# hyperledger-labs/bdls

Measured on AMD Instinct MI355X. Metric: P-256 ECDSA verifies/sec (fused SHA-256, bit-exact vs Go crypto/ecdsa + Fabric low-S), higher is better.
Workload: dtype u32; 1 GPU; BASELINE config 2: 1048576 records/GPU, 256B messages, 65536 distinct keys, 1/16 corrupted, fused SHA-256; records_per_gpu=1048576, records_total=1048576, msg_len=256, nkeys=65536, corrupt_den=16, parallelism=shard1 (no collective)

## Files before the change

### bdls_amd/csrc/bdls_hip.cpp

```cpp
#include <hip/hip_runtime.h>

#include <algorithm>
#include <cctype>
#include <atomic>
#include <chrono>
#include <condition_variable>
#include <deque>
#include <memory>
#include <cstdio>
#include <cstdlib>
#include <cstring>
#include <functional>
#include <mutex>
#include <string>
#include <unordered_map>
#include <thread>
#include <vector>

#include "../../include/bdls_hip.h"
#include "verify.h"
#include "verify384.h"
#include "pack.h"
#include "shard.h"

// ... 448 lines not shown

std::vector<Dev*> all_devs() {
  std::lock_guard<std::mutex> g(g_mu);
  return g_devs;
}

uint32_t env_block(const char* name, uint32_t dflt) {
  const char* e = getenv(name);
  const long v = e ? atol(e) : 0L;
  return (v == 64 || v == 128 || v == 256) ? (uint32_t)v : dflt;
}

int env_route() {
  const char* e = getenv("BH_ROUTE");
  if (!e) return 0;
  if (!strcmp(e, "ladder")) return 2;
  if (!strcmp(e, "noreg")) return 1;
  return 0;
}

bh::LaunchOpts launch_opts(size_t m, uint32_t flags) {
  bh::LaunchOpts o;
  static const long env_chunk = [] {
    const char* e = getenv("BH_INV_CHUNK");
    return e ? atol(e) : 0L;
  }();
  o.inv_chunk = env_chunk > 0 ? (uint32_t)std::min<long>(env_chunk, 64)
                              : (uint32_t)std::max<size_t>(1, std::min<size_t>(16, m / 131072));
  o.keep = (flags & BH_F_KEEP_KEYS) != 0;
  o.min_uses = o.keep ? 2u : bh::kMinUses;
  o.min_batch = o.keep ? 0u : bh::kKeyTableMinBatch;
  o.wide = bh::wide_for(m);
  o.wide_block = env_block("BH_WIDE_BLOCK", 256);
  return o;
}

bh::BatchIn slice(const bh_batch* b, size_t base, uint32_t flags) {
  return bh::BatchIn{b->pub + base * 64, b->sig, b->sig_off + base, b->sig_len + base,
                     b->msg, b->msg_off + base, b->msg_len + base, flags};
}
bh::BdlsIn slice(const bh_bdls_batch* b, size_t base, uint32_t flags) {
  return bh::BdlsIn{b->xy + base * 64, b->r, b->r_off + base, b->r_len + base,
                    b->s, b->s_off + base, b->s_len + base,
// ... 50 lines not shown
  }
  for (size_t base = 0; base < n; base += chunk) {
    const size_t m = std::min(chunk, n - base);
    bh::Work w;
    bh::Plan pl;
    int rc = carve_work(d, m, &w, &pl, false, lane > 0 ? L.ws : nullptr);
    if (rc) return rc;
    bh::LaunchOpts o = launch_opts(m, flags);
    {
      const char* e = getenv("BH_LL");
      o.ll_tables = !(e && atoi(e) == 0);
    }
    const int route = env_route();
    bh::KeyReg g = d.reg[curve].g;
    if (route >= 1 && !(flags & BH_F_KEEP_KEYS)) g.cap = 0;
    if (route >= 2 && !(flags & BH_F_KEEP_KEYS)) o.min_uses = UINT32_MAX;
    o.aux = L.aux;
    o.ev_fork = L.fork;
    o.ev_join = L.join;
    o.records_ready = records_ready;
    if (lane >= 0 && d.build_staggered && lanes() > 1) {
      const uint32_t nl = lanes();
      o.ev_build_wait = lane_ref(d, (int)((lane + nl - 1) % nl)).build;
      o.ev_build_done = L.build;
    }
    hipEvent_t* ev = t ? d.ev : nullptr;
    if (!t && d.defer) {
      if (d.ev_used == d.ev_pool.size()) {
        d.ev_pool.emplace_back(7, nullptr);
        for (auto& e : d.ev_pool.back()) HIPCHK(hipEventCreate(&e));
      }
// ... 1942 lines not shown
```

### bdls_amd/csrc/curve_consts.h

```cpp
#pragma once
#include <stdint.h>
namespace bh {
struct Fp_p256 {
  static constexpr uint32_t m[8] = {0xffffffffu, 0xffffffffu, 0xffffffffu, 0x00000000u, 0x00000000u, 0x00000000u, 0x00000001u, 0xffffffffu};
  static constexpr uint32_t n0 = 0x00000001u;
  static constexpr uint32_t r1[8] = {0x00000001u, 0x00000000u, 0x00000000u, 0xffffffffu, 0xffffffffu, 0xffffffffu, 0xfffffffeu, 0x00000000u};
  static constexpr uint32_t r2[8] = {0x00000003u, 0x00000000u, 0xffffffffu, 0xfffffffbu, 0xfffffffeu, 0xffffffffu, 0xfffffffdu, 0x00000004u};
  static constexpr uint32_t mm2[8] = {0xfffffffdu, 0xffffffffu, 0xffffffffu, 0x00000000u, 0x00000000u, 0x00000000u, 0x00000001u, 0xffffffffu};
  static constexpr uint32_t r3[8] = {0x0000000au, 0xfffffffdu, 0xfffffff7u, 0xffffffedu, 0xfffffffcu, 0x00000005u, 0x00000001u, 0x00000018u};
  static constexpr int32_t s30[9] = {1073741823, 1073741823, 1073741823, 63, 0, 0, 4096, 1073725440, 65535};
  static constexpr uint32_t inv30 = 0x3fffffffu;
};
struct Fn_p256 {
  static constexpr uint32_t m[8] = {0xfc632551u, 0xf3b9cac2u, 0xa7179e84u, 0xbce6faadu, 0xffffffffu, 0xffffffffu, 0x00000000u, 0xffffffffu};
  static constexpr uint32_t n0 = 0xee00bc4fu;
  static constexpr uint32_t r1[8] = {0x039cdaafu, 0x0c46353du, 0x58e8617bu, 0x43190552u, 0x00000000u, 0x00000000u, 0xffffffffu, 0x00000000u};
  static constexpr uint32_t r2[8] = {0xbe79eea2u, 0x83244c95u, 0x49bd6fa6u, 0x4699799cu, 0x2b6bec59u, 0x2845b239u, 0xf3d95620u, 0x66e12d94u};
  static constexpr uint32_t mm2[8] = {0xfc63254fu, 0xf3b9cac2u, 0xa7179e84u, 0xbce6faadu, 0xffffffffu, 0xffffffffu, 0x00000000u, 0xffffffffu};
  static constexpr uint32_t r3[8] = {0x0b65a624u, 0xac8ebec9u, 0x0c0555c9u, 0x111f28aeu, 0x6ba5e93fu, 0x2543b924u, 0x6407be65u, 0x503a54e7u};
  static constexpr int32_t s30[9] = {1013130577, 250030859, 830072911, 968797033, 1073741756, 1073741823, 4095, 1073725440, 65535};
  static constexpr uint32_t inv30 = 0x11ff43b1u;
};
struct Cv_p256 {
  static constexpr uint32_t b_m[8] = {0x29c4bddfu, 0xd89cdf62u, 0x78843090u, 0xacf005cdu, 0xf7212ed6u, 0xe5a220abu, 0x04874834u, 0xdc30061du};
// ... 9 lines not shown
  static constexpr uint32_t p[9] = {0x3fffffffu, 0x3fffffffu, 0x3fffffffu, 0x0000003fu, 0x00000000u, 0x00000000u, 0x00001000u, 0x3fffc000u, 0x0000ffffu};
  static constexpr uint32_t n0 = 0x00000001u;
  static constexpr uint32_t r1[9] = {0x00004000u, 0x00000000u, 0x00000000u, 0x3ff00000u, 0x3fffffffu, 0x3fffffffu, 0x3bffffffu, 0x0fffffffu, 0x00000000u};
  static constexpr uint32_t r2[9] = {0x30000000u, 0x00000000u, 0x00000000u, 0x3ffffffcu, 0x3fffffbfu, 0x3fffffbfu, 0x3fffffffu, 0x3ffff7ffu, 0x00004fffu};
  static constexpr uint32_t r3[9] = {0x00006000u, 0x0000a000u, 0x3fff4000u, 0x3fdfffffu, 0x3fb7ffffu, 0x3fcfffffu, 0x3b7fffffu, 0x18ffffffu, 0x00000000u};
  using M32 = Fp_p256;
  static constexpr uint32_t k32[9] = {0x7fffffe0u, 0x7ffffffeu, 0x7ffffffeu, 0x400007feu, 0x3fffffffu, 0x3fffffffu, 0x4001ffffu, 0x7ff7ffffu, 0x001ffffeu};
  static constexpr uint32_t k64[9] = {0x7fffffc0u, 0x7ffffffeu, 0x7ffffffeu, 0x40000ffeu, 0x3fffffffu, 0x3fffffffu, 0x4003ffffu, 0x7fefffffu, 0x003ffffeu};
  static constexpr uint32_t b_m[9] = {0x2f77f70cu, 0x1f6229c4u, 0x02436273u, 0x1cc9c543u, 0x35ab3c01u, 0x2bf7212eu, 0x1025c882u, 0x1e0b7483u, 0x00000187u};
  static constexpr uint32_t gx_m[9] = {0x050f0624u, 0x30d418a9u, 0x1805e79cu, 0x1fc475dbu, 0x041d6ea5u, 0x2b776225u, 0x1985adccu, 0x2bdc755cu, 0x000017ddu};
  static constexpr uint32_t gy_m[9] = {0x1582a15cu, 0x1357ce95u, 0x117377c9u, 0x0e434a9eu, 0x0962d2aeu, 0x08dd21f3u, 0x1535e21au, 0x0aaf85d8u, 0x00007fc6u};
  static constexpr uint32_t pm2[8] = {0xfffffffdu, 0xffffffffu, 0xffffffffu, 0x00000000u, 0x00000000u, 0x00000000u, 0x00000001u, 0xffffffffu};
  static constexpr int a_is_minus3 = 1;
  static constexpr int sparse_p256 = 1;
};
struct Fp_k1 {
  static constexpr uint32_t m[8] = {0xfffffc2fu, 0xfffffffeu, 0xffffffffu, 0xffffffffu, 0xffffffffu, 0xffffffffu, 0xffffffffu, 0xffffffffu};
  static constexpr uint32_t n0 = 0xd2253531u;
  static constexpr uint32_t r1[8] = {0x000003d1u, 0x00000001u, 0x00000000u, 0x00000000u, 0x00000000u, 0x00000000u, 0x00000000u, 0x00000000u};
  static constexpr uint32_t r2[8] = {0x000e90a1u, 0x000007a2u, 0x00000001u, 0x00000000u, 0x00000000u, 0x00000000u, 0x00000000u, 0x00000000u};
  static constexpr uint32_t mm2[8] = {0xfffffc2du, 0xfffffffeu, 0xffffffffu, 0xffffffffu, 0xffffffffu, 0xffffffffu, 0xffffffffu, 0xffffffffu};
  static constexpr uint32_t r3[8] = {0x3795f671u, 0x002bb1e3u, 0x00000b73u, 0x00000001u, 0x00000000u, 0x00000000u, 0x00000000u, 0x00000000u};
  static constexpr int32_t s30[9] = {1073740847, 1073741819, 1073741823, 1073741823, 1073741823, 1073741823, 1073741823, 1073741823, 65535};
  static constexpr uint32_t inv30 = 0x2ddacacfu;
};
struct Fn_k1 {
  static constexpr uint32_t m[8] = {0xd0364141u, 0xbfd25e8cu, 0xaf48a03bu, 0xbaaedce6u, 0xfffffffeu, 0xffffffffu, 0xffffffffu, 0xffffffffu};
  static constexpr uint32_t n0 = 0x5588b13fu;
  static constexpr uint32_t r1[8] = {0x2fc9bebfu, 0x402da173u, 0x50b75fc4u, 0x45512319u, 0x00000001u, 0x00000000u, 0x00000000u, 0x00000000u};
  static constexpr uint32_t r2[8] = {0x67d7d140u, 0x896cf214u, 0x0e7cf878u, 0x741496c2u, 0x5bcd07c6u, 0xe697f5e4u, 0x81c69bc5u, 0x9d671cd5u};
// ... 16 lines not shown
  static constexpr uint32_t p[9] = {0x3ffffc2fu, 0x3ffffffbu, 0x3fffffffu, 0x3fffffffu, 0x3fffffffu, 0x3fffffffu, 0x3fffffffu, 0x3fffffffu, 0x0000ffffu};
  static constexpr uint32_t n0 = 0x12253531u;
  static constexpr uint32_t r1[9] = {0x00f44000u, 0x00010000u, 0x00000000u, 0x00000000u, 0x00000000u, 0x00000000u, 0x00000000u, 0x00000000u, 0x00000000u};
  static constexpr uint32_t r2[9] = {0x10000000u, 0x0003a428u, 0x000007a2u, 0x00000004u, 0x00000000u, 0x00000000u, 0x00000000u, 0x00000000u, 0x00000000u};
  static constexpr uint32_t r3[9] = {0x00000000u, 0x1f671000u, 0x2c78cde5u, 0x0b73002bu, 0x00040000u, 0x00000000u, 0x00000000u, 0x00000000u, 0x00000000u};
  using M32 = Fp_k1;
  static constexpr uint32_t k32[9] = {0x7fff85e0u, 0x7fffff7eu, 0x7ffffffeu, 0x7ffffffeu, 0x7ffffffeu, 0x7ffffffeu, 0x7ffffffeu, 0x7ffffffeu, 0x001ffffeu};
  static constexpr uint32_t k64[9] = {0x7fff0bc0u, 0x7ffffefeu, 0x7ffffffeu, 0x7ffffffeu, 0x7ffffffeu, 0x7ffffffeu, 0x7ffffffeu, 0x7ffffffeu, 0x003ffffeu};
  static constexpr uint32_t b_m[9] = {0x06adc000u, 0x00070000u, 0x00000000u, 0x00000000u, 0x00000000u, 0x00000000u, 0x00000000u, 0x00000000u, 0x00000000u};
  static constexpr uint32_t gx_m[9] = {0x08b83460u, 0x2e5ae1feu, 0x1b6f5cd8u, 0x15329bc6u, 0x2708c78au, 0x0033fd12u, 0x225e7d23u, 0x3e9089f4u, 0x00007990u};
  static constexpr uint32_t gy_m[9] = {0x2bbe38ffu, 0x26d3a317u, 0x1936c57au, 0x15d1f1dcu, 0x0da37f17u, 0x1aac19c1u, 0x19c2dad6u, 0x3d4a582du, 0x0000e147u};
  static constexpr uint32_t pm2[8] = {0xfffffc2du, 0xfffffffeu, 0xffffffffu, 0xffffffffu, 0xffffffffu, 0xffffffffu, 0xffffffffu, 0xffffffffu};
  static constexpr int a_is_minus3 = 0;
  static constexpr int sparse_p256 = 0;
};
}
```

### bdls_amd/csrc/ec30.h

```cpp
#pragma once
#include "fp30.h"

namespace bh {

struct J30 {
  uint32_t X[9], Y[9], Z[9];
};

BH_HD void j_copy(J30& r, const J30& p) {
  f_copy(r.X, p.X);
  f_copy(r.Y, p.Y);
  f_copy(r.Z, p.Z);
}

BH_HD void j_sel(J30& r, bool c, const J30& a, const J30& b) {
  f_sel(r.X, c, a.X, b.X);
  f_sel(r.Y, c, a.Y, b.Y);
  f_sel(r.Z, c, a.Z, b.Z);
}

template <class F>
BH_HD void j_dbl(J30& r, const J30& p) {
  if constexpr (F::a_is_minus3) {
    uint32_t delta[9], gamma[9], bt[9], t0[9], t1[9], u[9], alpha[9];
// ... 101 lines not shown
  f_mul<F>(w1, p.X, c);
  f_mul<F>(w2, q.X, c);
  f_sub<F, 64>(t2, p.Y, q.Y);
  f_sqr<F>(d, t2);
  f_sub<F, 32>(t3, w1, w2);
  f_mul<F>(p.Y, p.Y, t3);
  f_sub2<F, 32>(r.X, d, w1, w2);
  f_sub<F, 64>(t3, w1, r.X);
  f_mul<F>(t3, t2, t3);
  f_sub<F, 32>(r.Y, t3, p.Y);
  f_mul<F>(r.Z, p.Z, t1);
  f_copy(p.X, w1);
  f_copy(p.Z, r.Z);
}

template <class F>
BH_HD bool j_degenerate(const uint32_t z3[9], const uint32_t rr[9], bool* same_y) {
  const bool degenerate = f_is_zero2<F>(z3);
  if (degenerate) {
    uint32_t t[9];
    f_reduce<F>(t, rr);
    uint32_t z = 0;
    for (int i = 0; i < 9; i++) z |= t[i];
    *same_y = (z == 0);
  } else {
    *same_y = false;
  }
  return degenerate;
}

template <class F, bool CO>
BH_HD bool j_add_impl(J30& r, J30* pz, const J30& p, const J30& q, bool neg, bool* same_y) {
  uint32_t z1z1[9], z2z2[9], u1[9], u2[9], s1[9], s2[9], h[9], rr[9], t[9], hh[9], hhh[9], w[9];
// ... 24 lines not shown
    f_copy(pz->Y, s1);
    f_copy(pz->Z, r.Z);
  }
  return j_degenerate<F>(r.Z, rr, same_y);
}

template <class F>
BH_HD bool j_add(J30& r, const J30& p, const J30& q, bool* same_y) {
  return j_add_impl<F, false>(r, nullptr, p, q, false, same_y);
}
template <class F>
BH_HD bool j_add_co(J30& r, J30& pz, const J30& p, const J30& q, bool* same_y, bool neg = false) {
  return j_add_impl<F, true>(r, &pz, p, q, neg, same_y);
}

template <class F, bool CO>
BH_HD bool j_madd_impl(J30& r, J30* pz, const J30& p, const uint32_t x2[9], const uint32_t y2[9],
                       bool neg, bool* same_y) {
  uint32_t z1z1[9], u2[9], s2[9], h[9], rr[9], t[9], hh[9], hhh[9], v[9], w[9];
  f_sqr<F>(z1z1, p.Z);
  f_mul<F>(u2, x2, z1z1);
  f_mul<F>(t, p.Z, z1z1);
  f_mul<F>(s2, y2, t);
  f_sub<F, 64>(h, u2, p.X);
  f_csub<F, 96>(rr, neg, s2, p.Y);
  f_sqr<F>(hh, h);
  f_mul<F>(hhh, hh, h);
  f_mul<F>(v, p.X, hh);
  f_sqr<F>(t, rr);
  f_add2x(w, hhh, v);
  f_sub<F, 32>(r.X, t, w);
  f_addsub<F, 32>(s2, w, v, t);
  f_mul<F>(s2, rr, s2);
  f_mul<F>(t, p.Y, hhh);
  f_sub<F, 32>(r.Y, s2, t);
  f_mul<F>(r.Z, p.Z, h);
  if constexpr (CO) {
    f_copy(pz->X, v);
    f_copy(pz->Y, t);
    f_copy(pz->Z, r.Z);
  }
  return j_degenerate<F>(r.Z, rr, same_y);
}

template <class F>
BH_HD bool j_madd(J30& r, const J30& p, const uint32_t x2[9], const uint32_t y2[9], bool* same_y,
                  bool neg = false) {
  return j_madd_impl<F, false>(r, nullptr, p, x2, y2, neg, same_y);
}
template <class F>
BH_HD bool j_madd_co(J30& r, J30& pz, const J30& p, const uint32_t x2[9], const uint32_t y2[9],
                     bool* same_y, bool neg = false) {
  return j_madd_impl<F, true>(r, &pz, p, x2, y2, neg, same_y);
}

template <class F>
BH_HD bool j_on_curve(const uint32_t x[9], const uint32_t y[9]) {
  uint32_t l[9], rhs[9], t[9], b[9];
  f_sqr<F>(l, y);
  f_sqr<F>(t, x);
  f_mul<F>(rhs, t, x);
  if constexpr (F::a_is_minus3) {
    f_mulc<3>(t, x);
    f_sub<F, 32>(rhs, rhs, t);
  }
  f_const(b, F::b_m);
  f_add(rhs, rhs, b);
  f_reduce<F>(rhs, rhs);
// ... 6 lines not shown
```

### bdls_amd/csrc/fp30.h

```cpp
#pragma once
#include "bh_common.h"
#include "curve_consts.h"

#ifndef BH_ZFILTER
#define BH_ZFILTER 0
#endif

namespace bh {

constexpr uint32_t kM30 = 0x3fffffffu;
constexpr int kL = 9;

BH_HD void f_copy(uint32_t r[9], const uint32_t a[9]) {
#pragma unroll
  for (int i = 0; i < 9; i++) r[i] = a[i];
}

BH_HD void f_sel(uint32_t r[9], bool c, const uint32_t a[9], const uint32_t b[9]) {
#pragma unroll
  for (int i = 0; i < 9; i++) r[i] = c ? a[i] : b[i];
}

template <class C>
BH_HD void f_const(uint32_t r[9], const C& c) {
// ... 224 lines not shown
template <class F>
BH_HD void f_reduce(uint32_t r[9], const uint32_t a[9]) {
  uint32_t one[9];
  f_const(one, F::r1);
  f_mul<F>(r, a, one);
  f_canon<F>(r, r);
}

BH_HD bool f_eq(const uint32_t a[9], const uint32_t b[9]) {
  uint32_t x = 0;
#pragma unroll
  for (int i = 0; i < 9; i++) x |= a[i] ^ b[i];
  return x == 0;
}

template <class F>
BH_HD bool f_is_zero2(const uint32_t a[9]) {
#if BH_ZFILTER
  if (a[0] != 0u && a[0] != F::p[0]) return false;
#endif
  uint32_t z = 0, q = 0;
#pragma unroll
  for (int i = 0; i < 9; i++) {
    z |= a[i];
    q |= a[i] ^ F::p[i];
  }
  return z == 0 || q == 0;
}

BH_HD void f_from_u256(uint32_t r[9], const uint32_t a[8]) {
  r[0] = a[0] & kM30;
#pragma unroll
  for (int i = 1; i < 8; i++) {
    const int lo = 30 * i;
    const int w = lo >> 5, s = lo & 31;
// ... 78 lines not shown
```

### bdls_amd/csrc/gen_consts.py

```python
#!/usr/bin/env python3
import sys

CURVES = {
    "p256": dict(
        p=2**256 - 2**224 + 2**192 + 2**96 - 1,
        n=0xFFFFFFFF00000000FFFFFFFFFFFFFFFFBCE6FAADA7179E84F3B9CAC2FC632551,
        a=-3,
        b=0x5AC635D8AA3A93E7B3EBBD55769886BC651D06B0CC53B0F63BCE3C3E27D2604B,
        gx=0x6B17D1F2E12C4247F8BCE6E563A440F277037D812DEB33A0F4A13945D898C296,
        gy=0x4FE342E2FE1A7F9B8EE7EB4A7C0F9E162BCE33576B315ECECBB6406837BF51F5,
    ),
    "k1": dict(
        p=2**256 - 2**32 - 977,
        n=0xFFFFFFFFFFFFFFFFFFFFFFFFFFFFFFFEBAAEDCE6AF48A03BBFD25E8CD0364141,
        a=0,
        b=7,
        gx=0x79BE667EF9DCBBAC55A06295CE870B07029BFCDB2DCE28D959F2815B16F81798,
        gy=0x483ADA7726A3C4655DA4FBFC0E1108A8FD17B448A68554199C47D08FFB10D4B8,
    ),
}
R = 2**256


def limbs(v):
# ... 47 lines not shown
    print(f"  static constexpr uint32_t r1[9] = {{{limbs30(R30 % p)}}};  // R mod p")
    print(f"  static constexpr uint32_t r2[9] = {{{limbs30(R30 * R30 % p)}}};  // R^2 mod p")
    print(f"  static constexpr uint32_t r3[9] = {{{limbs30(R30 ** 3 % p)}}};  // R^3 mod p (safegcd inverse)")
    print(f"  using M32 = Fp_{name[4:]};  // the same field on 32-bit limbs (fe.h safegcd)")
    print(f"  static constexpr uint32_t k32[9] = {{{borrowed30(32 * p)}}};  // 32p, borrowed form")
    print(f"  static constexpr uint32_t k64[9] = {{{borrowed30(64 * p)}}};  // 64p, borrowed form")
    print(f"  static constexpr uint32_t b_m[9] = {{{limbs30(c['b'] * R30 % p)}}};  // b R mod p")
    print(f"  static constexpr uint32_t gx_m[9] = {{{limbs30(c['gx'] * R30 % p)}}};")
    print(f"  static constexpr uint32_t gy_m[9] = {{{limbs30(c['gy'] * R30 % p)}}};")
    print(f"  static constexpr uint32_t pm2[8] = {{{limbs(p - 2)}}};  // Fermat exponent (32-bit limbs)")
    print(f"  static constexpr int a_is_minus3 = {1 if c['a'] == -3 else 0};")
    print(f"  static constexpr int sparse_p256 = {1 if p == 2**256 - 2**224 + 2**192 + 2**96 - 1 else 0};")
    print("};")


def main():
    print("// GENERATED by gen_consts.py -- do not edit.")
    print("#pragma once")
    print("#include <stdint.h>")
    print("namespace bh {")
    for cname, c in CURVES.items():
        emit_mod(f"Fp_{cname}", c["p"])
        emit_mod(f"Fn_{cname}", c["n"])
        p = c["p"]
        print(f"struct Cv_{cname} {{")
        print(f"  static constexpr uint32_t b_m[8] = {{{limbs(c['b'] * R % p)}}};  // b*R mod p")
        print(f"  static constexpr uint32_t gx_m[8] = {{{limbs(c['gx'] * R % p)}}};")
        print(f"  static constexpr uint32_t gy_m[8] = {{{limbs(c['gy'] * R % p)}}};")
        print(f"  static constexpr uint32_t half_n[8] = {{{limbs(c['n'] >> 1)}}};  // floor(n/2)")
        print(f"  static constexpr uint32_t p_minus_n[8] = {{{limbs(p - c['n'])}}};  // p - n")
        print(f"  static constexpr uint32_t n[8] = {{{limbs(c['n'])}}};")
        print(f"  static constexpr uint32_t p[8] = {{{limbs(p)}}};")
        print(f"  static constexpr int a_is_minus3 = {1 if c['a'] == -3 else 0};")
        print("};")
        emit_fp30(f"F30_{cname}", c)
    print("}  // namespace bh")


P384 = dict(
    p=2**384 - 2**128 - 2**96 + 2**32 - 1,
    n=0xFFFFFFFFFFFFFFFFFFFFFFFFFFFFFFFFFFFFFFFFFFFFFFFFC7634D81F4372DDF581A0DB248B0A77AECEC196ACCC52973,
    a=-3,
    b=0xB3312FA7E23EE7E4988E056BE3F82D19181D9C6EFE8141120314088F5013875AC656398D8A2ED19D2A85C8EDD3EC2AEF,
    gx=0xAA87CA22BE8B05378EB1C71EF320AD746E1D3B628BA79B9859F741E082542A385502F25DBF55296C3A545E3872760AB7,
    gy=0x3617DE4A96262C6F5D9E98BF9292DC29F8F41DBD289A147CE9DA3113B5F0B8C00A60B1CE1D7E819D7A431D7C90EA0E5F,
)
W28 = 28
L28 = 14
R28 = 2**(W28 * L28)
KP_MAX = 32
# ... 52 lines not shown
```

### bdls_amd/csrc/verify.h

```cpp
#pragma once
#include <type_traits>

#include "blake2b.h"
#include "der.h"
#include "fe.h"
#include "ec30.h"
#include "sha256.h"
#include "sha3.h"

namespace bh {

enum : uint32_t {
  BHF_HASH_SHA256 = 1u,
  BHF_NO_LOW_S = 2u,
  BHF_HASH_SHA3_256 = 8u,
  BHF_BDLS_PREHASHED = 0x100u,
};

enum : int { HK_GIVEN_OR_SHA256 = 0, HK_SHA3_256 = 1 };

enum : uint8_t { ST_R2OK = 0x80u };

struct BatchIn {
  const uint8_t* pub;
// ... 58 lines not shown
constexpr uint32_t kNone = 0xffffffffu;

struct LaunchOpts {
  uint32_t inv_chunk;
  uint32_t min_uses;
  uint32_t min_batch;
  bool keep;
  int wide;
  uint32_t wide_block = 256;
  void* aux = nullptr;
  void* ev_fork = nullptr;
  void* ev_join = nullptr;
  void* ev_build_wait = nullptr;
  void* ev_build_done = nullptr;
  bool ll_tables = true;
  void* records_ready = nullptr;
};

constexpr uint32_t kWide16Max = 8192, kWide4Max = 32768;
BH_HD int wide_for(size_t m) { return m <= kWide16Max ? 16 : m <= kWide4Max ? 4 : 1; }
BH_HD size_t gpart_slots(size_t ns) {
  const int wide = wide_for(ns);
  return wide > 1 ? (2 + (size_t)wide) * ns : ns;
}

#ifndef BH_GCOMB_BITS
#define BH_GCOMB_BITS 13
#endif
constexpr int kGW = BH_GCOMB_BITS;
static_assert(kGW >= 8 && kGW <= 14, "G comb window width");
// ... 135 lines not shown
    load_const8(pmn, C::p_minus_n);
    f_from_u256(rm, r);
    f_to_mont<P>(rm, rm);
    f_canon<P>(rm, rm);
    if (!geq8(r, pmn)) {
      st |= ST_R2OK;
      add8(rn, r, nn);
      f_from_u256(r2m, rn);
      f_to_mont<P>(r2m, r2m);
      f_canon<P>(r2m, r2m);
    } else {
      f_copy(r2m, rm);
    }
    st9(w.rm, i, w.ns, rm);
    st9(w.r2m, i, w.ns, r2m);
    to_mont<N>(s, s);
  } else {
    for (int k = 0; k < 8; k++) { e[k] = r[k] = 0; }
    e[0] = r[0] = 1;
    load_const8(s, N::r1);
    f_const(qx30, P::gx_m);
    f_const(qy30, P::gy_m);
  }
  if (!DEFER) st8(w.e, i, w.ns, e);
  st8(w.r, i, w.ns, r);
  st8(w.sm, i, w.ns, s);
  st9(w.qx, i, w.ns, qx30);
  st9(w.qy, i, w.ns, qy30);
  w.st[i] = st;
}

BH_HD void setbytes_u256(const uint8_t* b, uint32_t len, uint32_t v[8], bool* big, bool* zero) {
  uint32_t lo = 0;
  while (lo < len && b[lo] == 0) lo++;
  const uint32_t L = len - lo;
// ... 65 lines not shown
    load_const8(pmn, C::p_minus_n);
    f_from_u256(rm, r);
    f_to_mont<P>(rm, rm);
    f_canon<P>(rm, rm);
    if (!geq8(r, pmn)) {
      st |= ST_R2OK;
      add8(rn, r, nn);
      f_from_u256(r2m, rn);
      f_to_mont<P>(r2m, r2m);
      f_canon<P>(r2m, r2m);
    } else {
      f_copy(r2m, rm);
    }
    st9(w.rm, i, w.ns, rm);
    st9(w.r2m, i, w.ns, r2m);
    to_mont<N>(s, s);
  } else {
    for (int k = 0; k < 8; k++) r[k] = 0;
    r[0] = 1;
    load_const8(s, N::r1);
    f_const(qx30, P::gx_m);
    f_const(qy30, P::gy_m);
  }
  st8(w.r, i, w.ns, r);
  st8(w.sm, i, w.ns, s);
  st9(w.qx, i, w.ns, qx30);
  st9(w.qy, i, w.ns, qy30);
  w.st[i] = st;
}

template <class N, bool U1 = true, bool VAR = false>
BH_HD void stage_inv(const Work& w, uint32_t c, uint32_t stride, uint32_t n) {
  uint32_t acc[8], x[8];
  load_const8(acc, N::r1);
  uint32_t last = c;
  for (uint32_t i = c; i < n; i += stride) {
    st8(w.pre, i, w.ns, acc);
    ld8(x, w.sm, i, w.ns);
    mont_mul<N>(acc, acc, x);
    last = i;
  }
  if (c >= n) return;
  uint32_t inv[8];
  mont_inv_sg<N, VAR>(inv, acc);
  for (uint32_t i = last;; i -= stride) {
    uint32_t pre[8], wi[8], t[8];
    ld8(pre, w.pre, i, w.ns);
    mont_mul<N>(wi, inv, pre);
    ld8(x, w.sm, i, w.ns);
    mont_mul<N>(inv, inv, x);
    if constexpr (U1) {
      ld8(t, w.e, i, w.ns);
      mont_mul<N>(t, t, wi);
      st8(w.e, i, w.ns, t);
    } else {
      st8(w.sm, i, w.ns, wi);
    }
    ld8(t, w.r, i, w.ns);
    mont_mul<N>(t, t, wi);
    st8(w.r, i, w.ns, t);
    if (i < c + stride) break;
  }
}

template <class N>
BH_HD void calc_u1(uint32_t u1[8], const Work& w, uint32_t i) {
  uint32_t wi[8];
  ld8(u1, w.e, i, w.ns);
  ld8(wi, w.sm, i, w.ns);
  mont_mul<N>(u1, u1, wi);
}

BH_HD void booth5(uint32_t in6, uint32_t* mag, bool* neg) {
  uint32_t sgn = 0u - (in6 >> 5);
  uint32_t d = (63u - in6) & sgn;
  d |= in6 & ~sgn;
  *mag = (d >> 1) + (d & 1u);
  *neg = sgn != 0;
}


BH_HD uint32_t* qtab_entry(uint32_t* tab, uint32_t wave, uint32_t entry, uint32_t lane) {
  return tab + (((size_t)wave * 64 + lane) * kQTab + entry) * kQPt;
}

// ... 1071 lines not shown
#pragma unroll
  for (int cc = 0; cc < kGF; cc++) {
    uint32_t b = 0;
#pragma unroll
    for (int t = 0; t < kLLTeeth; t++) b |= (uint32_t)((gl[t] >> (j + cc)) & 1ull) << t;
    col[cc] = b;
  }
  neg = ((col[kGF - 1] >> (kLLTeeth - 1)) & 1u) == 0u;
  uint32_t x = col[kGF - 1] & (all >> 1);
  if (neg) x = ~col[kGF - 1] & (all >> 1);
#pragma unroll
  for (int cc = kGF - 2; cc >= 0; cc--) x = (x << kLLTeeth) | ((neg ? ~col[cc] : col[cc]) & all);
  idx = x;
}

template <class P>
BH_HD void ll_madd(J30& A, bool& a_inf, const uint32_t tx[9], uint32_t ty[9], bool neg,
                   const uint32_t one[9]) {
  bool same;
  const bool deg = j_madd<P>(A, A, tx, ty, &same, neg);
  if (a_inf || deg) {
    if (neg) f_neg<P, 64>(ty, ty);
    if (a_inf || same) {
      J30 T;
      f_copy(T.X, tx);
      f_copy(T.Y, ty);
      f_copy(T.Z, one);
      if (a_inf) j_copy(A, T);
      else j_dbl<P>(A, T);
      a_inf = false;
    } else {
      a_inf = true;
    }
  }
}

template <class P>
BH_HD void ll_dbladd(J30& A, bool& a_inf, const uint32_t tx[9], uint32_t ty[9], bool neg,
                     const uint32_t one[9]) {
  if (a_inf) {
    if (neg) f_neg<P, 64>(ty, ty);
    f_copy(A.X, tx);
    f_copy(A.Y, ty);
    f_copy(A.Z, one);
    a_inf = false;
    return;
  }
  J30 R, Az;
  bool same;
  if (j_madd_co<P>(R, Az, A, tx, ty, &same, neg)) {
    if (neg) f_neg<P, 64>(ty, ty);
    J30 T;
    f_copy(T.X, tx);
    f_copy(T.Y, ty);
    f_copy(T.Z, one);
    if (same) {
      j_dbl<P>(A, T);
      (void)j_madd<P>(A, A, tx, ty, &same);
    }
    return;
  }
  j_zaddu<P>(A, R, Az);
  if (f_is_zero2<P>(A.Z)) a_inf = true;
}

template <class P>
BH_HD void q_llcomb_g(J30& A, bool& a_inf, const Work& w, uint32_t i, const uint32_t* tab,
                      uint32_t stride, const uint32_t* g2) {
  uint32_t u2[8], u1[8], one[9];
  ld8(u2, w.r, i, w.ns);
  ld8(u1, w.e, i, w.ns);
  f_const(one, P::r1);
  uint64_t sl[kLLTeeth], gl[kLLTeeth];
  ll_slices<P>(sl, u2);
  ll_slices<P>(gl, u1);
  uint32_t idx;
  bool neg;
  ll_column(sl, kLLSpace - 1, idx, neg);
  if (stride) llent_load(A.X, A.Y, tab + idx * stride);
  else llaff_load(A.X, A.Y, tab, idx);
  f_copy(A.Z, one);
  a_inf = false;
  uint32_t gx[9], gy[9], gidx;
  bool gneg;
  g2_column(gl, kLLSpace - kGF, gidx, gneg);
  llaff_load(gx, gy, g2, gidx);
#pragma unroll 1
  for (int j = kLLSpace - 2; j >= 0; j--) {
    {
      uint32_t tx[9], ty[9];
      ll_column(sl, j, idx, neg);
      if (stride) llent_load(tx, ty, tab + idx * stride);
      else llaff_load(tx, ty, tab, idx);
      ll_dbladd<P>(A, a_inf, tx, ty, neg, one);
    }
    if (j == 0 || (j - 1) % kGF == 0) {
      ll_madd<P>(A, a_inf, gx, gy, gneg, one);
      if (j > 0) {
        g2_column(gl, j > kGF ? j - kGF : 0, gidx, gneg);
        llaff_load(gx, gy, g2, gidx);
      }
    }
  }
}

template <class P>
BH_HD bool stage_keycomb_fold(const Work& w, uint32_t i, const uint32_t* tab, uint32_t stride,
                              const uint32_t* g2) {
  J30 A;
  bool a_inf;
  q_llcomb_g<P>(A, a_inf, w, i, tab, stride, g2);
  return finish_check<P>(w, i, A, a_inf, A, true);
}

#ifndef BH_LADDER_CSUB
#define BH_LADDER_CSUB 1
#endif
template <class P>
BH_HD void j_dbladd(J30& A, bool& a_inf, J30& T, bool neg) {
  if (a_inf) {
    if (neg) f_neg<P, 64>(T.Y, T.Y);
    j_copy(A, T);
    a_inf = false;
    return;
  }
  J30 R, Az;
// ... 411 lines not shown
```

### bdls_amd/csrc/verify_kernels.hip

```cpp
#include <algorithm>
#include <type_traits>

#include <hipcub/hipcub.hpp>

#include "verify.h"

using namespace bh;

namespace {

template <class P, class N, class C, class IN, int HK, bool DEFER = false>
__global__ __launch_bounds__(256) void k_prep(IN in, Work w, uint32_t n) {
  const uint32_t i = blockIdx.x * blockDim.x + threadIdx.x;
  if (i >= n) return;
  if constexpr (std::is_same_v<IN, BatchIn>) stage_prep<P, N, C, HK, DEFER>(in, w, i);
  else stage_prep<P, N, C>(in, w, i);
}

template <class P, class C>
__global__ __launch_bounds__(256) void k_prep_keys(BatchIn in, Work w, uint32_t n) {
  const uint32_t i = blockIdx.x * blockDim.x + threadIdx.x;
  if (i >= n) return;
  stage_prep_key<P, C>(in, w, i);
}
// ... 625 lines not shown
}

#ifdef BH_KEYCOMB_WAVES
#define BH_KEYCOMB_ATTR __attribute__((amdgpu_waves_per_eu(BH_KEYCOMB_WAVES, BH_KEYCOMB_WAVES)))
#else
#define BH_KEYCOMB_ATTR
#endif
#ifndef BH_KEYCOMB_LDS
#define BH_KEYCOMB_LDS 1
#endif
#ifndef BH_LDS_TABS
#define BH_LDS_TABS ((17u * 64u) / kLLEnt)
#endif
constexpr uint32_t kLdsTabs = BH_LDS_TABS;
constexpr uint32_t kLdsTabWords = kLLEnt * kLLLds;
template <class P>
__global__ __launch_bounds__(256) BH_KEYCOMB_ATTR void k_keycomb(Work w, Plan pl, KeyReg g,
                                                 const uint32_t* __restrict__ gtab,
                                                 uint8_t* __restrict__ reason, uint32_t ll) {
  const uint32_t j = blockIdx.x * blockDim.x + threadIdx.x;
  const uint32_t cnt = pl.counters[0];
  if (!BH_KEYCOMB_LDS || !ll) {
    if (j >= cnt) return;
    const uint32_t i = pl.comb_order[j];
    const uint32_t id = pl.rec_tab[i];
    const bool ok = ll ? stage_keycomb_fold<P>(w, i, tab_ptr(pl, g, id), kLLAff, g2_of(gtab))
                       : stage_keycomb_q<P>(w, i, j, tab_ptr(pl, g, id), false, 0u,
                                            !(id & kLocal));
    reason[i] = ok ? R_OK : R_MATH;
    return;
  }
  if (blockIdx.x * blockDim.x >= cnt) return;
  __shared__ uint32_t s_tab[kLdsTabs * kLdsTabWords];
  __shared__ const uint32_t* s_src[kLdsTabs];
  __shared__ uint32_t s_id[256];
  __shared__ uint32_t s_wsum[4];
  const uint32_t t = threadIdx.x, lane = t & 63u, wv = t >> 6;
  const bool have = j < cnt;
  uint32_t i = 0, id = kNone;
  if (have) {
    i = pl.comb_order[j];
// ... 18 lines not shown
  if (start && slot < kLdsTabs) s_src[slot] = tab_ptr(pl, g, id);
  __syncthreads();
  const uint32_t nst = runs < kLdsTabs ? runs : kLdsTabs;
  for (uint32_t e = t; e < nst * kLLEnt; e += 256u) {
    const W4* s = reinterpret_cast<const W4*>(s_src[e / kLLEnt] + (e % kLLEnt) * kLLAff);
    const W4 a = s[0], b = s[1], c = s[2], d = s[3], f = s[4];
    W2* o = reinterpret_cast<W2*>(s_tab + e * kLLLds);
    o[0] = W2{a.x, a.y}; o[1] = W2{a.z, a.w}; o[2] = W2{b.x, b.y};
    o[3] = W2{b.z, b.w}; o[4] = W2{c.x, c.y}; o[5] = W2{c.z, c.w};
    o[6] = W2{d.x, d.y}; o[7] = W2{d.z, d.w}; o[8] = W2{f.x, f.y};
  }
  __syncthreads();
  if (!have) return;
  const bool in_lds = lcl && slot < kLdsTabs;
  const uint32_t* tab = in_lds ? s_tab + slot * kLdsTabWords : tab_ptr(pl, g, id);
  const bool ok = stage_keycomb_fold<P>(w, i, tab, in_lds ? kLLLds : kLLAff, g2_of(gtab));
  reason[i] = ok ? R_OK : R_MATH;
}

template <class P, int L>
__global__ __launch_bounds__(256) void k_keycomb_wide(Work w, Plan pl, KeyReg g,
                                                      const uint32_t* __restrict__ gtab,
                                                      uint8_t* __restrict__ reason) {
  const uint32_t gid = blockIdx.x * blockDim.x + threadIdx.x;
  const uint32_t j = gid / L, l = gid % L;
  const uint32_t cnt = pl.counters[0];
  if (j >= cnt) return;
  const uint32_t i = pl.comb_order[j];
  const uint32_t id = pl.rec_tab[i];
  J30 C;
  bool c_inf;
  keycomb_part<P, L>(C, c_inf, w, gtab, i, tab_ptr(pl, g, id), l, !(id & kLocal));
// ... 384 lines not shown
      const uint32_t tb = (pl.max_tables + kBuildPerBlock - 1) / kBuildPerBlock;
      if (o.ev_build_wait && (e = hipStreamWaitEvent(s, (hipEvent_t)o.ev_build_wait, 0)))
        return e;
      hipLaunchKernelGGL((k_ktab_ladder<P>), dim3(tb), blk, 0, s, w, pl, g, gtab, reason, tb, 0u,
                         1u);
      if (o.ev_build_done && (e = hipEventRecord((hipEvent_t)o.ev_build_done, s))) return e;
      if ((e = hipStreamWaitEvent(s, (hipEvent_t)o.records_ready, 0))) return e;
      launch_prep<P, N, C>(in, w, n, grd, blk, s);
      hipLaunchKernelGGL((k_inv<N, true>), grc, blk, 0, s, w, n, nlanes);
      hipLaunchKernelGGL(k_split, dim3((n + kSplitBlock - 1) / kSplitBlock), dim3(kSplitBlock), 0,
                         s, w, pl, n, reason);
      Plan plk;
      if ((e = comb_sort(pl, g, n, s, &plk))) return e;
      hipLaunchKernelGGL((k_ktab_ladder<P>), grd, blk, 0, s, w, plk, g, gtab, reason, 0u, grd.x,
                         1u);
      hipLaunchKernelGGL((k_keycomb<P>), grd, blk, 0, s, w, plk, g, gtab, reason, 1u);
      hipLaunchKernelGGL(k_bitmap, grd, blk, 0, s, reason, n, bitmap);
      return hipGetLastError();
    }
  }
  bool joined = true;
  hipStream_t hs = s;
  if ((kBdls || split) && o.aux) {
    hs = (hipStream_t)o.aux;
    if ((e = hipEventRecord((hipEvent_t)o.ev_fork, s))) return e;
    if ((e = hipStreamWaitEvent(hs, (hipEvent_t)o.ev_fork, 0))) return e;
    joined = false;
  }
  if constexpr (kBdls) {
    if (in.flags & BHF_BDLS_PREHASHED)
      hipLaunchKernelGGL((k_bdls_given<C>), grd, blk, 0, hs, in, w, n);
// ... 93 lines not shown
  if (o.ev_build_done && (e = hipEventRecord((hipEvent_t)o.ev_build_done, s))) return e;
  REC(4);
  if (o.keep)
    hipLaunchKernelGGL(k_reg_publish, dim3((pl.max_tables + 255) / 256), blk, 0, s, w, plc, g);
  REC(5);
  switch (o.wide) {
    case 4:
      hipLaunchKernelGGL((k_keycomb_wide<P, 4>), wgrd(n * 4), wblk, 0, s, w, plc, g,
                         gtab, reason);
      break;
    case 16:
      hipLaunchKernelGGL((k_keycomb_wide<P, 16>), wgrd(n * 16), wblk, 0, s, w, plc,
                         g, gtab, reason);
      break;
    default:
      hipLaunchKernelGGL((k_keycomb<P>), grd, blk, 0, s, w, plc, g, gtab, reason, ll);
  }
  hipLaunchKernelGGL(k_bitmap, grd, blk, 0, s, reason, n, bitmap);
  REC(6);
#undef REC
  return hipGetLastError();
}

hipError_t launch_verify(int curve, const BatchIn& in, const Work& w, const Plan& pl,
                         const KeyReg& g, const uint32_t* gtab, uint32_t n, const LaunchOpts& o,
                         uint64_t* bitmap, uint8_t* reason, hipStream_t s, hipEvent_t* ev) {
  if (curve != 0) return hipErrorInvalidValue;
  return seq<F30_p256, Fn_p256, Cv_p256>(in, w, pl, g, gtab, n, o, bitmap, reason, s, ev);
}

hipError_t launch_verify_bdls(int curve, const BdlsIn& in, const Work& w, const Plan& pl,
// ... 51 lines not shown
```

Before: 187.0 million verifies/s.

## Move scalar batch inversion to radix-2^30, add wave zero-filter, raise inv chunk

The batched modular inversion of s (prefix products and back-substitution) now runs on 9-limb radix-2^30 Montgomery arithmetic for the group order instead of the 8x32 Montgomery path. It also drops the to_mont conversion and uses new Fn30 constants. A wave-level ballot early-out for the degenerate Z==0 check is added to the comb kernel, controlled by a runtime flag that defaults on. The default inversion chunk rises to 32 for batches of a million or more, and a 'comb' route option is added. Together these aim to cut multiply cost and branch work in inversion and comb addition, at the price of extra limb conversions on every load and store.

```diff
diff --git a/bdls_amd/csrc/bdls_hip.cpp b/bdls_amd/csrc/bdls_hip.cpp
--- a/bdls_amd/csrc/bdls_hip.cpp
+++ b/bdls_amd/csrc/bdls_hip.cpp
@@ -486,6 +486,7 @@
 int env_route() {
   const char* e = getenv("BH_ROUTE");
   if (!e) return 0;
+  if (!strcmp(e, "comb")) return 3;
   if (!strcmp(e, "ladder")) return 2;
   if (!strcmp(e, "noreg")) return 1;
   return 0;
@@ -493,12 +494,16 @@
 
 bh::LaunchOpts launch_opts(size_t m, uint32_t flags) {
   bh::LaunchOpts o;
-  static const long env_chunk = [] {
-    const char* e = getenv("BH_INV_CHUNK");
-    return e ? atol(e) : 0L;
-  }();
-  o.inv_chunk = env_chunk > 0 ? (uint32_t)std::min<long>(env_chunk, 64)
-                              : (uint32_t)std::max<size_t>(1, std::min<size_t>(16, m / 131072));
+  constexpr size_t kInvChunkBig = 32;
+  const char* ce = getenv("BH_INV_CHUNK");
+  const long env_chunk = ce ? atol(ce) : 0L;
+  const size_t dflt = m >= ((size_t)1 << 20) ? kInvChunkBig
+                                             : std::max<size_t>(1, std::min<size_t>(16, m / 131072));
+  o.inv_chunk = env_chunk > 0 ? (uint32_t)std::min<long>(env_chunk, 64) : (uint32_t)dflt;
+  {
+    const char* e = getenv("BH_COMB_ZFILTER");
+    o.comb_zfilter = !(e && atoi(e) == 0);
+  }
   o.keep = (flags & BH_F_KEEP_KEYS) != 0;
   o.min_uses = o.keep ? 2u : bh::kMinUses;
   o.min_batch = o.keep ? 0u : bh::kKeyTableMinBatch;
@@ -579,7 +584,11 @@
     const int route = env_route();
     bh::KeyReg g = d.reg[curve].g;
     if (route >= 1 && !(flags & BH_F_KEEP_KEYS)) g.cap = 0;
-    if (route >= 2 && !(flags & BH_F_KEEP_KEYS)) o.min_uses = UINT32_MAX;
+    if (route == 2 && !(flags & BH_F_KEEP_KEYS)) o.min_uses = UINT32_MAX;
+    if (route == 3 && !(flags & BH_F_KEEP_KEYS)) {
+      o.wide = 1;
+      o.min_batch = 0;
+    }
     o.aux = L.aux;
     o.ev_fork = L.fork;
     o.ev_join = L.join;
diff --git a/bdls_amd/csrc/curve_consts.h b/bdls_amd/csrc/curve_consts.h
--- a/bdls_amd/csrc/curve_consts.h
+++ b/bdls_amd/csrc/curve_consts.h
@@ -47,6 +47,14 @@
   static constexpr int a_is_minus3 = 1;
   static constexpr int sparse_p256 = 1;
 };
+struct Fn30_p256 {
+  static constexpr uint32_t p[9] = {0x3c632551u, 0x0ee72b0bu, 0x3179e84fu, 0x39beab69u, 0x3fffffbcu, 0x3fffffffu, 0x00000fffu, 0x3fffc000u, 0x0000ffffu};
+  static constexpr uint32_t n0 = 0x2e00bc4fu;
+  static constexpr uint32_t r1[9] = {0x36abc000u, 0x353d039cu, 0x05ec3118u, 0x15258e86u, 0x0010c641u, 0x00000000u, 0x3c000000u, 0x0fffffffu, 0x00000000u};
+  static constexpr uint32_t r2[9] = {0x0887ac57u, 0x05d911a5u, 0x130785e0u, 0x2a328ab8u, 0x19076a9eu, 0x1afb1658u, 0x2484a92bu, 0x2a0ebf05u, 0x000055abu};
+  using M32 = Fn_p256;
+  static constexpr int sparse_p256 = 0;
+};
 struct Fp_k1 {
   static constexpr uint32_t m[8] = {0xfffffc2fu, 0xfffffffeu, 0xffffffffu, 0xffffffffu, 0xffffffffu, 0xffffffffu, 0xffffffffu, 0xffffffffu};
   static constexpr uint32_t n0 = 0xd2253531u;
@@ -93,4 +101,12 @@
   static constexpr int a_is_minus3 = 0;
   static constexpr int sparse_p256 = 0;
 };
+struct Fn30_k1 {
+  static constexpr uint32_t p[9] = {0x10364141u, 0x3f497a33u, 0x348a03bbu, 0x2bb739abu, 0x3ffffebau, 0x3fffffffu, 0x3fffffffu, 0x3fffffffu, 0x0000ffffu};
+  static constexpr uint32_t n0 = 0x1588b13fu;
+  static constexpr uint32_t r1[9] = {0x2fafc000u, 0x21732fc9u, 0x3f1100b6u, 0x31950b75u, 0x00515448u, 0x00000000u, 0x00000000u, 0x00000000u, 0x00000000u};
+  static constexpr uint32_t r2[9] = {0x3c6a0df3u, 0x090ea30du, 0x103606edu, 0x17c0c584u, 0x01a618aeu, 0x3341f1cfu, 0x17f5e45bu, 0x1a6f179au, 0x0000581cu};
+  using M32 = Fn_k1;
+  static constexpr int sparse_p256 = 0;
+};
 }
diff --git a/bdls_amd/csrc/ec30.h b/bdls_amd/csrc/ec30.h
--- a/bdls_amd/csrc/ec30.h
+++ b/bdls_amd/csrc/ec30.h
@@ -139,9 +139,9 @@
   f_copy(p.Z, r.Z);
 }
 
-template <class F>
+template <class F, bool ZF = false>
 BH_HD bool j_degenerate(const uint32_t z3[9], const uint32_t rr[9], bool* same_y) {
-  const bool degenerate = f_is_zero2<F>(z3);
+  const bool degenerate = f_is_zero2<F, ZF>(z3);
   if (degenerate) {
     uint32_t t[9];
     f_reduce<F>(t, rr);
@@ -196,7 +196,7 @@
   return j_add_impl<F, true>(r, &pz, p, q, neg, same_y);
 }
 
-template <class F, bool CO>
+template <class F, bool CO, bool ZF = false>
 BH_HD bool j_madd_impl(J30& r, J30* pz, const J30& p, const uint32_t x2[9], const uint32_t y2[9],
                        bool neg, bool* same_y) {
   uint32_t z1z1[9], u2[9], s2[9], h[9], rr[9], t[9], hh[9], hhh[9], v[9], w[9];
@@ -222,18 +222,18 @@
     f_copy(pz->Y, t);
     f_copy(pz->Z, r.Z);
   }
-  return j_degenerate<F>(r.Z, rr, same_y);
-}
-
-template <class F>
+  return j_degenerate<F, ZF>(r.Z, rr, same_y);
+}
+
+template <class F, bool ZF = false>
 BH_HD bool j_madd(J30& r, const J30& p, const uint32_t x2[9], const uint32_t y2[9], bool* same_y,
                   bool neg = false) {
-  return j_madd_impl<F, false>(r, nullptr, p, x2, y2, neg, same_y);
-}
-template <class F>
+  return j_madd_impl<F, false, ZF>(r, nullptr, p, x2, y2, neg, same_y);
+}
+template <class F, bool ZF = false>
 BH_HD bool j_madd_co(J30& r, J30& pz, const J30& p, const uint32_t x2[9], const uint32_t y2[9],
                      bool* same_y, bool neg = false) {
-  return j_madd_impl<F, true>(r, &pz, p, x2, y2, neg, same_y);
+  return j_madd_impl<F, true, ZF>(r, &pz, p, x2, y2, neg, same_y);
 }
 
 template <class F>
diff --git a/bdls_amd/csrc/fp30.h b/bdls_amd/csrc/fp30.h
--- a/bdls_amd/csrc/fp30.h
+++ b/bdls_amd/csrc/fp30.h
@@ -1,10 +1,6 @@
 #pragma once
 #include "bh_common.h"
 #include "curve_consts.h"
-
-#ifndef BH_ZFILTER
-#define BH_ZFILTER 0
-#endif
 
 namespace bh {
 
@@ -262,11 +258,16 @@
   return x == 0;
 }
 
-template <class F>
+template <class F, bool ZF = false>
 BH_HD bool f_is_zero2(const uint32_t a[9]) {
-#if BH_ZFILTER
-  if (a[0] != 0u && a[0] != F::p[0]) return false;
+  if constexpr (ZF) {
+    const bool maybe = a[0] == 0u || a[0] == F::p[0];
+#if defined(__HIP_DEVICE_COMPILE__)
+    if (__builtin_amdgcn_ballot_w64(maybe) == 0ull) return false;
+#else
+    if (!maybe) return false;
 #endif
+  }
   uint32_t z = 0, q = 0;
 #pragma unroll
   for (int i = 0; i < 9; i++) {
diff --git a/bdls_amd/csrc/gen_consts.py b/bdls_amd/csrc/gen_consts.py
--- a/bdls_amd/csrc/gen_consts.py
+++ b/bdls_amd/csrc/gen_consts.py
@@ -85,6 +85,18 @@
     print("};")
 
 
+def emit_fn30(name, cname, n):
+    n0 = (-pow(n, -1, 2**W)) % 2**W
+    print(f"struct {name} {{  // the group order n in radix 2^30, R = 2^270")
+    print(f"  static constexpr uint32_t p[9] = {{{limbs30(n)}}};")
+    print(f"  static constexpr uint32_t n0 = 0x{n0:08x}u;  // -n^-1 mod 2^30")
+    print(f"  static constexpr uint32_t r1[9] = {{{limbs30(R30 % n)}}};  // R mod n")
+    print(f"  static constexpr uint32_t r2[9] = {{{limbs30(R30 * R30 % n)}}};  // R^2 mod n")
+    print(f"  using M32 = Fn_{cname};  // the same field on 32-bit limbs (fe.h safegcd)")
+    print("  static constexpr int sparse_p256 = 0;")
+    print("};")
+
+
 def main():
     print("// GENERATED by gen_consts.py -- do not edit.")
     print("#pragma once")
@@ -105,6 +117,7 @@
         print(f"  static constexpr int a_is_minus3 = {1 if c['a'] == -3 else 0};")
         print("};")
         emit_fp30(f"F30_{cname}", c)
+        emit_fn30(f"Fn30_{cname}", cname, c["n"])
     print("}  // namespace bh")
 
 
diff --git a/bdls_amd/csrc/verify.h b/bdls_amd/csrc/verify.h
--- a/bdls_amd/csrc/verify.h
+++ b/bdls_amd/csrc/verify.h
@@ -96,6 +96,7 @@
   void* ev_build_wait = nullptr;
   void* ev_build_done = nullptr;
   bool ll_tables = true;
+  bool comb_zfilter = true;
   void* records_ready = nullptr;
 };
 
@@ -261,11 +262,9 @@
     }
     st9(w.rm, i, w.ns, rm);
     st9(w.r2m, i, w.ns, r2m);
-    to_mont<N>(s, s);
   } else {
-    for (int k = 0; k < 8; k++) { e[k] = r[k] = 0; }
-    e[0] = r[0] = 1;
-    load_const8(s, N::r1);
+    for (int k = 0; k < 8; k++) { e[k] = r[k] = s[k] = 0; }
+    e[0] = r[0] = s[0] = 1;
     f_const(qx30, P::gx_m);
     f_const(qy30, P::gy_m);
   }
@@ -361,11 +360,9 @@
     }
     st9(w.rm, i, w.ns, rm);
     st9(w.r2m, i, w.ns, r2m);
-    to_mont<N>(s, s);
   } else {
-    for (int k = 0; k < 8; k++) r[k] = 0;
-    r[0] = 1;
-    load_const8(s, N::r1);
+    for (int k = 0; k < 8; k++) r[k] = s[k] = 0;
+    r[0] = s[0] = 1;
     f_const(qx30, P::gx_m);
     f_const(qy30, P::gy_m);
   }
@@ -376,46 +373,74 @@
   w.st[i] = st;
 }
 
+template <class N>
+using N30Of = typename std::conditional<std::is_same<N, Fn_p256>::value, Fn30_p256, Fn30_k1>::type;
+
+BH_HD void ld8_30(uint32_t r[9], const uint32_t* base, uint32_t i, uint32_t ns) {
+  uint32_t t[8];
+  ld8(t, base, i, ns);
+  f_from_u256(r, t);
+}
+template <class F>
+BH_HD void st8_30(uint32_t* base, uint32_t i, uint32_t ns, const uint32_t a[9]) {
+  uint32_t c[9], t[8];
+  f_canon<F>(c, a);
+  f_to_u256(t, c);
+  st8(base, i, ns, t);
+}
+
 template <class N, bool U1 = true, bool VAR = false>
 BH_HD void stage_inv(const Work& w, uint32_t c, uint32_t stride, uint32_t n) {
-  uint32_t acc[8], x[8];
-  load_const8(acc, N::r1);
+  using F = N30Of<N>;
+  uint32_t acc[9], x[9];
+  f_const(acc, F::r1);
   uint32_t last = c;
   for (uint32_t i = c; i < n; i += stride) {
-    st8(w.pre, i, w.ns, acc);
-    ld8(x, w.sm, i, w.ns);
-    mont_mul<N>(acc, acc, x);
+    st8_30<F>(w.pre, i, w.ns, acc);
+    ld8_30(x, w.sm, i, w.ns);
+    f_mul<F>(acc, acc, x);
     last = i;
   }
   if (c >= n) return;
-  uint32_t inv[8];
-  mont_inv_sg<N, VAR>(inv, acc);
+  uint32_t inv[9];
+  {
+    uint32_t a8[8], i8[8], r2[9];
+    f_canon<F>(acc, acc);
+    f_to_u256(a8, acc);
+    mod_inv_sg<N, VAR>(i8, a8);
+    f_from_u256(inv, i8);
+    f_const(r2, F::r2);
+    f_mul<F>(inv, inv, r2);
+  }
   for (uint32_t i = last;; i -= stride) {
-    uint32_t pre[8], wi[8], t[8];
-    ld8(pre, w.pre, i, w.ns);
-    mont_mul<N>(wi, inv, pre);
-    ld8(x, w.sm, i, w.ns);
-    mont_mul<N>(inv, inv, x);
+    uint32_t pre[9], wi[9], t[9];
+    ld8_30(pre, w.pre, i, w.ns);
+    f_mul<F>(wi, inv, pre);
+    ld8_30(x, w.sm, i, w.ns);
+    f_mul<F>(inv, inv, x);
     if constexpr (U1) {
-      ld8(t, w.e, i, w.ns);
-      mont_mul<N>(t, t, wi);
-      st8(w.e, i, w.ns, t);
+      ld8_30(t, w.e, i, w.ns);
+      f_mul<F>(t, t, wi);
+      st8_30<F>(w.e, i, w.ns, t);
     } else {
-      st8(w.sm, i, w.ns, wi);
-    }
-    ld8(t, w.r, i, w.ns);
-    mont_mul<N>(t, t, wi);
-    st8(w.r, i, w.ns, t);
+      st8_30<F>(w.sm, i, w.ns, wi);
+    }
+    ld8_30(t, w.r, i, w.ns);
+    f_mul<F>(t, t, wi);
+    st8_30<F>(w.r, i, w.ns, t);
     if (i < c + stride) break;
   }
 }
 
 template <class N>
 BH_HD void calc_u1(uint32_t u1[8], const Work& w, uint32_t i) {
-  uint32_t wi[8];
-  ld8(u1, w.e, i, w.ns);
-  ld8(wi, w.sm, i, w.ns);
-  mont_mul<N>(u1, u1, wi);
+  using F = N30Of<N>;
+  uint32_t e[9], wi[9];
+  ld8_30(e, w.e, i, w.ns);
+  ld8_30(wi, w.sm, i, w.ns);
+  f_mul<F>(e, e, wi);
+  f_canon<F>(e, e);
+  f_to_u256(u1, e);
 }
 
 BH_HD void booth5(uint32_t in6, uint32_t* mag, bool* neg) {
@@ -1517,11 +1542,11 @@
   idx = x;
 }
 
-template <class P>
+template <class P, bool ZF = false>
 BH_HD void ll_madd(J30& A, bool& a_inf, const uint32_t tx[9], uint32_t ty[9], bool neg,
                    const uint32_t one[9]) {
   bool same;
-  const bool deg = j_madd<P>(A, A, tx, ty, &same, neg);
+  const bool deg = j_madd<P, ZF>(A, A, tx, ty, &same, neg);
   if (a_inf || deg) {
     if (neg) f_neg<P, 64>(ty, ty);
     if (a_inf || same) {
@@ -1538,7 +1563,7 @@
   }
 }
 
-template <class P>
+template <class P, bool ZF = false>
 BH_HD void ll_dbladd(J30& A, bool& a_inf, const uint32_t tx[9], uint32_t ty[9], bool neg,
                      const uint32_t one[9]) {
   if (a_inf) {
@@ -1551,7 +1576,7 @@
   }
   J30 R, Az;
   bool same;
-  if (j_madd_co<P>(R, Az, A, tx, ty, &same, neg)) {
+  if (j_madd_co<P, ZF>(R, Az, A, tx, ty, &same, neg)) {
     if (neg) f_neg<P, 64>(ty, ty);
     J30 T;
     f_copy(T.X, tx);
@@ -1564,10 +1589,10 @@
     return;
   }
   j_zaddu<P>(A, R, Az);
-  if (f_is_zero2<P>(A.Z)) a_inf = true;
-}
-
-template <class P>
+  if (f_is_zero2<P, ZF>(A.Z)) a_inf = true;
+}
+
+template <class P, bool ZF = false>
 BH_HD void q_llcomb_g(J30& A, bool& a_inf, const Work& w, uint32_t i, const uint32_t* tab,
                       uint32_t stride, const uint32_t* g2) {
   uint32_t u2[8], u1[8], one[9];
@@ -1595,10 +1620,10 @@
       ll_column(sl, j, idx, neg);
       if (stride) llent_load(tx, ty, tab + idx * stride);
       else llaff_load(tx, ty, tab, idx);
-      ll_dbladd<P>(A, a_inf, tx, ty, neg, one);
+      ll_dbladd<P, ZF>(A, a_inf, tx, ty, neg, one);
     }
     if (j == 0 || (j - 1) % kGF == 0) {
-      ll_madd<P>(A, a_inf, gx, gy, gneg, one);
+      ll_madd<P, ZF>(A, a_inf, gx, gy, gneg, one);
       if (j > 0) {
         g2_column(gl, j > kGF ? j - kGF : 0, gidx, gneg);
         llaff_load(gx, gy, g2, gidx);
@@ -1607,12 +1632,12 @@
   }
 }
 
-template <class P>
+template <class P, bool ZF = false>
 BH_HD bool stage_keycomb_fold(const Work& w, uint32_t i, const uint32_t* tab, uint32_t stride,
                               const uint32_t* g2) {
   J30 A;
   bool a_inf;
-  q_llcomb_g<P>(A, a_inf, w, i, tab, stride, g2);
+  q_llcomb_g<P, ZF>(A, a_inf, w, i, tab, stride, g2);
   return finish_check<P>(w, i, A, a_inf, A, true);
 }
 
diff --git a/bdls_amd/csrc/verify_kernels.hip b/bdls_amd/csrc/verify_kernels.hip
--- a/bdls_amd/csrc/verify_kernels.hip
+++ b/bdls_amd/csrc/verify_kernels.hip
@@ -663,7 +663,7 @@
 #endif
 constexpr uint32_t kLdsTabs = BH_LDS_TABS;
 constexpr uint32_t kLdsTabWords = kLLEnt * kLLLds;
-template <class P>
+template <class P, bool ZF>
 __global__ __launch_bounds__(256) BH_KEYCOMB_ATTR void k_keycomb(Work w, Plan pl, KeyReg g,
                                                  const uint32_t* __restrict__ gtab,
                                                  uint8_t* __restrict__ reason, uint32_t ll) {
@@ -673,7 +673,7 @@
     if (j >= cnt) return;
     const uint32_t i = pl.comb_order[j];
     const uint32_t id = pl.rec_tab[i];
-    const bool ok = ll ? stage_keycomb_fold<P>(w, i, tab_ptr(pl, g, id), kLLAff, g2_of(gtab))
+    const bool ok = ll ? stage_keycomb_fold<P, ZF>(w, i, tab_ptr(pl, g, id), kLLAff, g2_of(gtab))
                        : stage_keycomb_q<P>(w, i, j, tab_ptr(pl, g, id), false, 0u,
                                             !(id & kLocal));
     reason[i] = ok ? R_OK : R_MATH;
@@ -722,8 +722,16 @@
   if (!have) return;
   const bool in_lds = lcl && slot < kLdsTabs;
   const uint32_t* tab = in_lds ? s_tab + slot * kLdsTabWords : tab_ptr(pl, g, id);
-  const bool ok = stage_keycomb_fold<P>(w, i, tab, in_lds ? kLLLds : kLLAff, g2_of(gtab));
+  const bool ok = stage_keycomb_fold<P, ZF>(w, i, tab, in_lds ? kLLLds : kLLAff, g2_of(gtab));
   reason[i] = ok ? R_OK : R_MATH;
+}
+
+template <class P>
+static void launch_keycomb(bool zf, dim3 grd, dim3 blk, hipStream_t s, const Work& w,
+                           const Plan& pl, const KeyReg& g, const uint32_t* gtab, uint8_t* reason,
+                           uint32_t ll) {
+  if (zf) hipLaunchKernelGGL((k_keycomb<P, true>), grd, blk, 0, s, w, pl, g, gtab, reason, ll);
+  else hipLaunchKernelGGL((k_keycomb<P, false>), grd, blk, 0, s, w, pl, g, gtab, reason, ll);
 }
 
 template <class P, int L>
@@ -1138,7 +1146,7 @@
       if ((e = comb_sort(pl, g, n, s, &plk))) return e;
       hipLaunchKernelGGL((k_ktab_ladder<P>), grd, blk, 0, s, w, plk, g, gtab, reason, 0u, grd.x,
                          1u);
-      hipLaunchKernelGGL((k_keycomb<P>), grd, blk, 0, s, w, plk, g, gtab, reason, 1u);
+      launch_keycomb<P>(o.comb_zfilter, grd, blk, s, w, plk, g, gtab, reason, 1u);
       hipLaunchKernelGGL(k_bitmap, grd, blk, 0, s, reason, n, bitmap);
       return hipGetLastError();
     }
@@ -1262,7 +1270,7 @@
                          g, gtab, reason);
       break;
     default:
-      hipLaunchKernelGGL((k_keycomb<P>), grd, blk, 0, s, w, plc, g, gtab, reason, ll);
+      launch_keycomb<P>(o.comb_zfilter, grd, blk, s, w, plc, g, gtab, reason, ll);
   }
   hipLaunchKernelGGL(k_bitmap, grd, blk, 0, s, reason, n, bitmap);
   REC(6);
```

New measurement: 189.3 million verifies/s (median of 6 runs). 1.2% higher.
